# yanrui89/LearningAgileFlight_SE3

Hardware: AMD Instinct MI355X
Metric: MPC solves+gradients/sec (batch, 50-step horizon) at 1/2/4/8 MI355X (higher is better)
Workload: dtype f64

## Files before the change

### learningagileflight_se3_amd/csrc/ipm_kernel.hip

```cpp
#include <hip/hip_runtime.h>

#include <cstdint>

#include "lafse3.h"
#include "model.hpp"
#include "weight_columns.hpp"
#include "riccati_tables.hpp"

namespace lafse3 {

typedef __attribute__((address_space(1))) double gdouble;
typedef double dvec2 __attribute__((ext_vector_type(2)));
typedef __attribute__((address_space(1))) dvec2 gdvec2;

constexpr int MAXN = LAFSE3_MAX_N;
constexpr int SX = MAXN + 1;
constexpr int PST = 18;
constexpr int GST = 22;
constexpr int FMAX = 64;
constexpr int WAVE = 64;
__device__ inline int lane_id() { return (int)(threadIdx.x & (WAVE - 1)); }
__device__ inline int64_t slot_id() { return (int64_t)blockIdx.x; }
constexpr int TRACE_W = 16;
constexpr int DUMP_STEP_W = (MAXN + 1) * NX + MAXN * NU + MAXN * NX;
constexpr int DUMP_W = 2 * DUMP_STEP_W + 2 * MAXN * NU + 2 * (MAXN + 1) * 3;
static_assert(DUMP_W == 3732, "lafse3.h documents the dump record as 3732 doubles per instance");
constexpr int RD_STEP_W = DUMP_STEP_W + 2 * MAXN * NX;
constexpr int RD_POINT_W = DUMP_W - DUMP_STEP_W + 4 * MAXN * NX;
constexpr int RD_REF_W = (MAXN + 1) * NX + MAXN * NU;
constexpr int RD_NSCAL = 6;
constexpr int RD_SCAL = RD_STEP_W + RD_POINT_W + RD_REF_W;
constexpr int RD_LSQ = RD_SCAL + RD_NSCAL;
constexpr int RD_W = RD_LSQ + MAXN * NX + 2;
static_assert(RD_W == 9153, "lafse3.h documents the restoration dump record as 9153 doubles per instance");

enum Mode : int { MODE_SOLVE = 0, MODE_OBJECTIVE = 1, MODE_GRAD = 2, MODE_GETINPUT = 3, MODE_REWARD = 4 };
enum { ST_SOLVED = 0, ST_ACCEPTABLE = 1, ST_MAXITER = 2, ST_LS_FAIL = 3, ST_NONFINITE = 4, ST_TINY = 5,
       ST_REG_FAIL = 6, ST_DEVICE_ERR = 7, ST_RESTO_FAIL = 8, ST_INFEASIBLE = 9 };
constexpr int CNT_ERR = 4;
constexpr int CNT_RESTO = 5;
constexpr int N_COUNTERS = 7;
enum : unsigned long long { ERR_PROBE_LOST = 1ull };

constexpr int WS_RQ = 0;
constexpr int WS_RR = WS_RQ + NX * SX;
constexpr int WS_RC = WS_RR + NU * SX;
constexpr int WS_BDX = WS_RC + NX * SX;
constexpr int WS_BDU = WS_BDX + NX * SX;
constexpr int WS_BLP = WS_BDU + NU * SX;
constexpr int BK_DX = 0, BK_DU = WS_BDU - WS_BDX, BK_LP = WS_BLP - WS_BDX;
constexpr int WS_TAB = WS_BLP + NX * SX;
constexpr int PSTR = NUP17 + 1;
constexpr int WS_PST = WS_TAB + MAXN * TB_W;
constexpr int WS_PN = WS_PST + MAXN * PSTR;
constexpr int WS_Z = WS_PN + 16;
constexpr int WS_CS = WS_Z + 14 * SX;
constexpr int WS_SDX = WS_CS + NX * SX;
constexpr int WS_SDU = WS_SDX + NX * SX;
constexpr int WS_SLP = WS_SDU + NU * SX;
constexpr int RC_K = 0, RC_KF = 4 * NA, RC_L = RC_KF + NU, REC = RC_L + 10;
static_assert(REC % 2 == 0, "record: whole 16-byte pieces");
constexpr int WS_REC = (WS_SLP + NX * SX + 1) & ~1;
constexpr int WS_KREF = WS_REC + MAXN * REC;
constexpr int WS_GS = WS_KREF + NU * SX;
constexpr int WS_PC = WS_GS + NU * SX;
constexpr int WS_RADJ = WS_PC + (MAXN + 1) * 18;
constexpr int WS_PVK = WS_RADJ + (MAXN + 1) * 16;
constexpr int WS_DX = WS_PVK + (MAXN + 1) * 18;
constexpr int WS_DU = WS_DX + NX * SX;
constexpr int WS_LAM = WS_DU + NU * SX;
constexpr int WS_LAMP = WS_LAM + NX * SX;
constexpr int WS_FILT = WS_LAMP + NX * SX;
#ifdef LAFSE3_FAC_CHECK
constexpr int WS_CHK = WS_FILT + 2 * FMAX;
constexpr int WS_END = WS_CHK + MAXN * (REC + PSTR) + (MAXN + 1) * 18;
#else
constexpr int WS_END = WS_FILT + 2 * FMAX;
#endif
constexpr int WS_SIZE0 = (WS_END + 15) & ~15;
constexpr int WS_SIZE = ((WS_SIZE0 / 16) % 2 == 0) ? WS_SIZE0 + 16 : WS_SIZE0;
constexpr int R_P = 0, R_N = R_P + NX * SX, R_ZP = R_N + NX * SX, R_ZN = R_ZP + NX * SX;
constexpr int R_DP = R_ZN + NX * SX, R_DN = R_DP + NX * SX, R_RP = R_DN + NX * SX, R_RN = R_RP + NX * SX;
constexpr int R_BP = R_RN + NX * SX, R_BN = R_BP + NX * SX, R_D = R_BN + NX * SX, R_C = R_D + NX * SX;
constexpr int R_XR = R_C + NX * SX, R_DX2 = R_XR + NX * SX, R_UR = R_DX2 + NX * SX, R_DU2 = R_UR + NU * SX;
constexpr int R_SLAM = R_DU2 + NU * SX, R_SZ = R_SLAM + NX * SX, R_FILT = R_SZ + 14 * SX;
constexpr int RS_L = 0, RS_SD = 91, RS_PK = RS_SD + NX, RS_PV = RS_PK + 91, RS_K = RS_PV + NX, RS_KF = RS_K + NU * NX;
constexpr int RS_STG = RS_KF + NU;
constexpr int R_STG = R_FILT + 2 * FMAX;
constexpr int R_WD = R_STG + MAXN * RS_STG;
constexpr int WD_X = 0, WD_U = WD_X + NX * SX, WD_LAM = WD_U + NU * SX, WD_Z = WD_LAM + NX * SX, WD_DX = WD_Z + 14 * SX;
constexpr int WD_DU = WD_DX + NX * SX, WD_LP = WD_DU + NU * SX, WD_SIZE = WD_LP + NX * SX;
constexpr int RWS_SIZE = (R_WD + WD_SIZE + 15) & ~15;
constexpr int RW_SIZE = 768;
constexpr int WS_ZLU = WS_Z, WS_ZUU = WS_Z + NU * SX, WS_ZLW = WS_Z + 2 * NU * SX, WS_ZUW = WS_Z + 2 * NU * SX + 3 * SX;
#define WS_TRAJ(ws)                                                                                          \
    [[maybe_unused]] double *DX = const_cast<double *>(S.dx), *DU = const_cast<double *>(S.du);              \
    [[maybe_unused]] double *LAM = const_cast<double *>(S.lam), *LP = const_cast<double *>(S.lamp);          \
    [[maybe_unused]] gdouble *ZLU = (gdouble *)(ws) + WS_ZLU, *ZUU = (gdouble *)(ws) + WS_ZUU;                 \
    [[maybe_unused]] gdouble *ZLW = (gdouble *)(ws) + WS_ZLW, *ZUW = (gdouble *)(ws) + WS_ZUW

struct KernelArgs {
    lafse3_params prm;
    int mode;
    int64_t n_inst;
    const double *ini, *goal, *gate12, *ptra, *atra, *t, *ulast;
    const float *dnn;
    const double *x_in;
    double *x_out, *u_out, *lam_out, *cost_out, *reward_out;
    int32_t *status_out, *iters_out;
    unsigned long long *counters;
    int persistent;
    unsigned *sched;
    double *trace;
    int trace_iters;
    unsigned long long *ptime;
    double *dump;
    int dump_it;
    int dump_refine;
    int64_t drop_push;
    double *ws;
    double *rws;
};

struct RestoDumpArgs {
    double *buf;
    int entry, it;
    int refine;
};
constexpr int REC_X = 0, REC_U = REC_X + (MAXN + 1) * NX, REC_LAM = REC_U + MAXN * NU, REC_ZLU = REC_LAM + MAXN * NX;
constexpr int REC_ZUU = REC_ZLU + MAXN * NU, REC_ZLW = REC_ZUU + MAXN * NU, REC_ZUW = REC_ZLW + (MAXN + 1) * 3;
constexpr int REC_MU = REC_ZUW + (MAXN + 1) * 3, REC_S = REC_MU + 1, REC_STATUS = REC_S + 1, REC_N = REC_STATUS + 1;
constexpr int REC_W = REC_N + 1;
static_assert(REC_MU == DUMP_W - DUMP_STEP_W, "the record's arrays are dump_point's iterate block");
static_assert(REC_W == 2223, "lafse3.h documents the optimum record as 2223 doubles per instance");
struct ExtArgs {
    const double *weights;
    double *dx_out, *du_out;
    double *gain_out;
    int32_t *sens_out;
    int32_t groups;
    double *rec;
};

struct Ctl {
    int N;
    double s;
    double mu;
    double ulo, uhi, wlo, whi;
};

constexpr int RING = 24;
constexpr int VGU = 44;
struct __align__(16) Smem {
    double x[NX * SX], u[NU * SX];
    double dx[NX * SX], du[NU * SX];
    double lam[NX * SX], lamp[NX * SX];
    alignas(16) double P[NA * PST];
    double p[24];
    union {
// ... 569 lines not shown
        double nr = 0.0;
        for (int r = 0; r < 1; ++r) nr = kkt_residual(M, at, S, C, ws, dw, soc);
        PT_END(S, 6);
        if (step < 0) {
            ratio = nr;
            ratios[0] = nr; ratios[1] = -1; ratios[2] = -1; ratios[3] = 0;
            continue;
        }
        if (step < 2) ratios[1 + step] = nr;
        ratios[3] += 1;
        if (!(nr < ratio)) {
            revert_to_backup(DX, LP, DU, bk, C.N);
            vm_sync();
            break;
        }
        ratio = nr;
    }
    return 1;
}

__device__ __noinline__ void soc_defects(const Model &M, const Smem &S, const Ctl &C, gdouble *ws, double alpha, int init)
{
    WS_TRAJ(ws);
    const int lane = lane_id();
    const int N = C.N;
    gdouble *cs = ws + WS_CS;
    if (lane < N) {
        const int k = lane;
        double xk[NX], uk[NU], xn[NX];
#pragma unroll
        for (int i = 0; i < NX; ++i) xk[i] = S.x[i * SX + k] + alpha * DX[i * SX + k];
#pragma unroll
        for (int a = 0; a < NU; ++a) uk[a] = S.u[a * SX + k] + alpha * DU[a * SX + k];
        f_disc(M, xk, uk, xn);
#pragma unroll
        for (int i = 0; i < NX; ++i) {
            const double ct = xn[i] - (S.x[i * SX + k + 1] + alpha * DX[i * SX + k + 1]);
            cs[i * SX + k] = init ? ct : alpha * cs[i * SX + k] + ct;
        }
    }
    vm_sync();
}

__device__ __noinline__ void soc_direction(const Model &M, const Attitude &at, Smem &S, const Ctl &C, gdouble *ws,
                                           double dw, int &sweeps)
{
    const int lane = lane_id();
    const int N = C.N;
    gdouble *rq = ws + WS_RQ, *rr = ws + WS_RR, *rc = ws + WS_RC;
    const gdouble *cs = ws + WS_CS;
    if (lane < N) {
        const int k = lane;
        double gu[NU];
        grad_u(M, S, C, k, gu);
#pragma unroll
        for (int a = 0; a < NU; ++a) {
            double gb, sg;
            bar_terms(S.u[a * SX + k], C.ulo, C.uhi, 0, 0, C.mu, gb, sg);
            rr[a * SX + k] = gu[a] + gb;
        }
        const int k1 = k + 1;
        double x1[NX], g[NX];
        load_stage(S, k1, x1);
        grad_x(M, at, S, C, k1, x1, g);
#pragma unroll
        for (int c = 0; c < 3; ++c) {
            double gb, sg;
            bar_terms(x1[10 + c], C.wlo, C.whi, 0, 0, C.mu, gb, sg);
            g[10 + c] += gb;
        }
#pragma unroll
        for (int i = 0; i < NX; ++i) {
            rq[i * SX + k1] = g[i];
            rc[i * SX + k] = cs[i * SX + k];
        }
    }
    vm_sync();
    double ratios[4] = {0, 0, 0, 0};
    linear_solve(M, at, S, C, ws, dw, 0, 0, 1, 1, sweeps, ratios, nullptr);
}

struct BoundDir {
    double du[NU], zlu[NU], zuu[NU], dw[3], zlw[3], zuw[3];
};
__device__ __attribute__((always_inline)) inline void load_bound_dir(const Smem &S, gdouble *ws, int k, BoundDir &b)
{
    WS_TRAJ(ws);
    const int k1 = k + 1;
#pragma unroll
    for (int a = 0; a < NU; ++a) {
        b.du[a] = DU[a * SX + k];
        b.zlu[a] = ZLU[a * SX + k];
        b.zuu[a] = ZUU[a * SX + k];
    }
#pragma unroll
    for (int c = 0; c < 3; ++c) {
        b.dw[c] = DX[(10 + c) * SX + k1];
        b.zlw[c] = ZLW[c * SX + k1];
        b.zuw[c] = ZUW[c * SX + k1];
    }
    __builtin_amdgcn_sched_barrier(0);
}

__device__ __noinline__ void frac_to_bound(const Smem &S, const Ctl &C, gdouble *ws, double tau, double mu, double &amax,
                                           double &az)
{
    WS_TRAJ(ws);
    const int lane = lane_id();
    const int N = C.N;
    double am = 1.0, a_z = 1.0;
    if (lane < N) {
        const int k = lane;
        const int k1 = k + 1;
        BoundDir bd;
        load_bound_dir(S, ws, k, bd);
#pragma unroll
        for (int a = 0; a < NU; ++a) {
            double v = S.u[a * SX + k], d = bd.du[a];
            double sl = v - C.ulo, su = C.uhi - v;
            if (d < 0) am = fmin(am, -tau * sl / d);
            if (d > 0) am = fmin(am, tau * su / d);
            double zl = bd.zlu[a], zu = bd.zuu[a];
            double dzl = mu / sl - zl - zl / sl * d;
            double dzu = mu / su - zu + zu / su * d;
            if (dzl < 0) a_z = fmin(a_z, -tau * zl / dzl);
            if (dzu < 0) a_z = fmin(a_z, -tau * zu / dzu);
        }
#pragma unroll
        for (int c = 0; c < 3; ++c) {
            double v = S.x[(10 + c) * SX + k1], d = bd.dw[c];
            double sl = v - C.wlo, su = C.whi - v;
            if (d < 0) am = fmin(am, -tau * sl / d);
            if (d > 0) am = fmin(am, tau * su / d);
            double zl = bd.zlw[c], zu = bd.zuw[c];
            double dzl = mu / sl - zl - zl / sl * d;
            double dzu = mu / su - zu + zu / su * d;
            if (dzl < 0) a_z = fmin(a_z, -tau * zl / dzl);
            if (dzu < 0) a_z = fmin(a_z, -tau * zu / dzu);
        }
    }
    amax = wmin(am);
    az = wmin(a_z);
}

struct DirStats {
    double amax, az, gBD, rel;
};
__device__ __noinline__ DirStats direction_stats(const Model &M, const Attitude &at, const Smem &S, const Ctl &C, gdouble *ws,
                                                 double tau, double mu)
{
    WS_TRAJ(ws);
    const int lane = lane_id();
    const int N = C.N;
double amax = 1.0, az = 1.0, gBD = 0.0, rel = 0.0;
    if (lane < N) {
        const int k = lane;
        BoundDir bd;
        load_bound_dir(S, ws, k, bd);
        double gu[NU];
        grad_u(M, S, C, k, gu);
#pragma unroll
        for (int a = 0; a < NU; ++a) {
            double v = S.u[a * SX + k], d = bd.du[a];
            double sl = v - C.ulo, su = C.uhi - v;
            if (d < 0) amax = fmin(amax, -tau * sl / d);
            if (d > 0) amax = fmin(amax, tau * su / d);
            double zl = bd.zlu[a], zu = bd.zuu[a];
            double dzl = mu / sl - zl - zl / sl * d;
            double dzu = mu / su - zu + zu / su * d;
            if (dzl < 0) az = fmin(az, -tau * zl / dzl);
            if (dzu < 0) az = fmin(az, -tau * zu / dzu);
            double gb, sg;
            bar_terms(v, C.ulo, C.uhi, 0, 0, mu, gb, sg);
            gBD += (gu[a] + gb) * d;
            rel = fmax(rel, fabs(d) / (1.0 + fabs(v)));
        }
        const int k1 = k + 1;
        double x1[NX], g[NX];
        load_stage(S, k1, x1);
        grad_x(M, at, S, C, k1, x1, g);
#pragma unroll
        for (int c = 0; c < 3; ++c) {
            double v = x1[10 + c], d = bd.dw[c];
            double sl = v - C.wlo, su = C.whi - v;
            if (d < 0) amax = fmin(amax, -tau * sl / d);
            if (d > 0) amax = fmin(amax, tau * su / d);
            double zl = bd.zlw[c], zu = bd.zuw[c];
            double dzl = mu / sl - zl - zl / sl * d;
            double dzu = mu / su - zu + zu / su * d;
            if (dzl < 0) az = fmin(az, -tau * zl / dzl);
            if (dzu < 0) az = fmin(az, -tau * zu / dzu);
            double gb, sg;
            bar_terms(v, C.wlo, C.whi, 0, 0, mu, gb, sg);
            g[10 + c] += gb;
        }
#pragma unroll
        for (int i = 0; i < NX; ++i) {
            double d = DX[i * SX + k1];
            gBD += g[i] * d;
            rel = fmax(rel, fabs(d) / (1.0 + fabs(x1[i])));
        }
    }
    amax = wmin(amax);
    az = wmin(az);
    gBD = wsum(gBD);
    rel = wmax(rel);
    DirStats D;
    D.amax = amax;
    D.az = az;
    D.gBD = gBD;
    D.rel = rel;
    return D;
}

__device__ __noinline__ void accept_step(Smem &S, const Ctl &C, gdouble *ws, double alpha, double az, double mu)
{
    WS_TRAJ(ws);
    const int lane = lane_id();
    const int N = C.N;
    if (lane < N) {
        const int k = lane, k1 = k + 1;
        double zlu_[NU], zuu_[NU], zlw_[3], zuw_[3];
#pragma unroll
        for (int a = 0; a < NU; ++a) {
            zlu_[a] = ZLU[a * SX + k];
            zuu_[a] = ZUU[a * SX + k];
        }
#pragma unroll
        for (int c = 0; c < 3; ++c) {
            zlw_[c] = ZLW[c * SX + k1];
            zuw_[c] = ZUW[c * SX + k1];
        }
#pragma unroll
        for (int a = 0; a < NU; ++a) {
            double v = S.u[a * SX + k], d = DU[a * SX + k];
            double sl = v - C.ulo, su = C.uhi - v;
            double zl = zlu_[a], zu = zuu_[a];
            zl = zl + az * (mu / sl - zl - zl / sl * d);
            zu = zu + az * (mu / su - zu + zu / su * d);
            v = v + alpha * d;
            S.u[a * SX + k] = v;
            sl = v - C.ulo;
            su = C.uhi - v;
            zlu_[a] = fmax(fmin(zl, 1e10 * mu / sl), mu / (1e10 * sl));
            zuu_[a] = fmax(fmin(zu, 1e10 * mu / su), mu / (1e10 * su));
        }
#pragma unroll
        for (int c = 0; c < 3; ++c) {
            double v = S.x[(10 + c) * SX + k1], d = DX[(10 + c) * SX + k1];
            double sl = v - C.wlo, su = C.whi - v;
            double zl = zlw_[c], zu = zuw_[c];
            zlw_[c] = zl + az * (mu / sl - zl - zl / sl * d);
            zuw_[c] = zu + az * (mu / su - zu + zu / su * d);
        }
        double lk[NX], lpk[NX], dx1[NX];
#pragma unroll
        for (int i = 0; i < NX; ++i) {
            lk[i] = LAM[i * SX + k];
            lpk[i] = LP[i * SX + k];
            dx1[i] = DX[i * SX + k1];
        }
#pragma unroll
        for (int i = 0; i < NX; ++i) {
            LAM[i * SX + k] = lk[i] + alpha * (lpk[i] - lk[i]);
            S.x[i * SX + k1] += alpha * dx1[i];
        }
#pragma unroll
        for (int c = 0; c < 3; ++c) {
            double v = S.x[(10 + c) * SX + k1];
            double sl = v - C.wlo, su = C.whi - v;
            double zl = zlw_[c], zu = zuw_[c];
            zlw_[c] = fmax(fmin(zl, 1e10 * mu / sl), mu / (1e10 * sl));
            zuw_[c] = fmax(fmin(zu, 1e10 * mu / su), mu / (1e10 * su));
        }
#pragma unroll
        for (int a = 0; a < NU; ++a) {
            ZLU[a * SX + k] = zlu_[a];
            ZUU[a * SX + k] = zuu_[a];
        }
#pragma unroll
        for (int c = 0; c < 3; ++c) {
            ZLW[c * SX + k1] = zlw_[c];
            ZUW[c * SX + k1] = zuw_[c];
        }
    }
    vm_sync();
}

static_assert(FMAX <= WAVE, "one filter entry per lane");
__device__ inline int filter_ok(const gdouble *FT, const gdouble *FP, int nfilt, double th, double ph)
{
    const int f = opaque_lane();
    double ft = 0.0, fp = 0.0;
    if (f < nfilt) {
        ft = FT[f];
        fp = FP[f];
    }
    return __ballot(f < nfilt && !(th <= ft || ph <= fp)) == 0ull;
}
__device__ inline int filter_add(gdouble *FT, gdouble *FP, int nfilt, double th0, double ph0)
{
    const int lane = opaque_lane();
    const double nt = (1.0 - 1e-5) * th0, np = ph0 - 1e-8 * th0;
    double ft = 0.0, fp = 0.0;
    if (lane < nfilt) {
        ft = FT[lane];
        fp = FP[lane];
    }
    const bool keep = lane < nfilt && !(ft >= nt && fp >= np);
    const unsigned long long m = __ballot(keep);
    int w = __popcll(m);
    if (keep) {
        const int pos = __popcll(m & ((1ull << lane) - 1ull));
        FT[pos] = ft;
        FP[pos] = fp;
    }
    if (w < FMAX) {
        if (lane == 0) {
            FT[w] = nt;
            FP[w] = np;
        }
        w++;
    }
    vm_sync();
    return w;
}

__device__ inline int ls_accept(const gdouble *FT, const gdouble *FP, int nfilt, double alpha_test, double tht, double pht, int okt, double th0,
                                double ph0, double gBD, double pg, double pt, double theta_max, double theta_min)
{
    const double eps = 2.220446049250313e-16;
    int acc = okt && !(tht > theta_max);
    if (acc) {
        int ftype = (gBD < 0) && (alpha_test * pg > pt);
        if (ftype && th0 <= theta_min) {
            acc = (pht - ph0 - 1e-8 * alpha_test * gBD) <= 10.0 * eps * fabs(ph0);
        } else {
            int objinc_ok = 1;
            if (pht > ph0) {
                double basval = (fabs(ph0) > 10.0) ? log10(fabs(ph0)) : 1.0;
                if (log10(pht - ph0) > 5.0 + basval) objinc_ok = 0;
            }
            acc = objinc_ok && (((tht - (1.0 - 1e-5) * th0) <= 10.0 * eps * fabs(th0)) ||
                                ((pht - ph0 + 1e-8 * th0) <= 10.0 * eps * fabs(ph0)));
        }
    }
    if (acc && !filter_ok(FT, FP, nfilt, tht, pht)) return 0;
    return acc;
}
__device__ inline int ls_accept(const gdouble *FT, const gdouble *FP, int nfilt, double alpha_test, double tht, double pht, int okt, double th0,
                                double ph0, double gBD, double theta_max, double theta_min)
{
    double pg = 0.0, pt = 0.0;
    if (okt && !(tht > theta_max) && gBD < 0) {
        pg = pow(-gBD, 2.3);
        pt = pow(th0, 1.1);
    }
    return ls_accept(FT, FP, nfilt, alpha_test, tht, pht, okt, th0, ph0, gBD, pg, pt, theta_max, theta_min);
}

struct Errs {
    double dinf, pinf, cmu, c0, sd, sc;
};

__device__ __attribute__((always_inline)) inline Errs compute_errors(const Model &M, const Attitude &at, const Smem &S, const Ctl &C, gdouble *ws,
                                            double mu)
{
    Errs E;
    WS_TRAJ(ws);
    const int lane = opaque_lane();
    const int N = C.N;
    double dinf = 0, pinf = 0, cmu = 0, c0 = 0, smult = 0, sz = 0;
    if (lane < N) {
        const int k = lane;
        double xk[NX], uk[NU], lk[NX];
        load_stage(S, k, xk);
        load_u(S, k, uk);
#pragma unroll
        for (int i = 0; i < NX; ++i) lk[i] = LAM[i * SX + k];
        double gu[NU], btl[NU];
        grad_u(M, S, C, k, gu);
        Bt_times(M, xk, lk, btl);
#pragma unroll
        for (int a = 0; a < NU; ++a) {
            double zl = ZLU[a * SX + k], zu = ZUU[a * SX + k];
            double acc = gu[a] + btl[a] - zl + zu;
            dinf = fmax(dinf, fabs(acc));
            double sl = uk[a] - C.ulo, su = C.uhi - uk[a];
            cmu = fmax(cmu, fmax(fabs(sl * zl - mu), fabs(su * zu - mu)));
            c0 = fmax(c0, fmax(fabs(sl * zl), fabs(su * zu)));
            sz += zl + zu;
        }
        double xn[NX];
        f_disc(M, xk, uk, xn);
#pragma unroll
        for (int i = 0; i < NX; ++i) {
            pinf = fmax(pinf, fabs(xn[i] - S.x[i * SX + k + 1]));
            smult += fabs(lk[i]);
        }
        const int k1 = k + 1;
        double x1[NX], g[NX];
        load_stage(S, k1, x1);
        grad_x(M, at, S, C, k1, x1, g);
#pragma unroll
        for (int i = 0; i < NX; ++i) g[i] -= lk[i];
        if (k1 < N) {
            double u1[NU], l1[NX], atl[NX];
            load_u(S, k1, u1);
#pragma unroll
            for (int i = 0; i < NX; ++i) l1[i] = LAM[i * SX + k1];
            At_times(M, x1, u1, l1, atl);
#pragma unroll
            for (int i = 0; i < NX; ++i) g[i] += atl[i];
        }
#pragma unroll
        for (int c = 0; c < 3; ++c) {
            double zl = ZLW[c * SX + k1], zu = ZUW[c * SX + k1];
            g[10 + c] += -zl + zu;
            double sl = x1[10 + c] - C.wlo, su = C.whi - x1[10 + c];
            cmu = fmax(cmu, fmax(fabs(sl * zl - mu), fabs(su * zu - mu)));
            c0 = fmax(c0, fmax(fabs(sl * zl), fabs(su * zu)));
            sz += zl + zu;
        }
#pragma unroll
        for (int i = 0; i < NX; ++i) dinf = fmax(dinf, fabs(g[i]));
    }
    dinf = wmax(dinf);
    pinf = wmax(pinf);
    cmu = wmax(cmu);
    c0 = wmax(c0);
    smult = wsum(smult);
    sz = wsum(sz);
    const double smax = 100.0;
    double n_mult = (double)(N * NX) + (double)(N * NU * 2 + N * 3 * 2);
    double n_z = (double)(N * NU * 2 + N * 3 * 2);
    E.sd = fmax(smax, (smult + sz) / n_mult) / smax;
    E.sc = fmax(smax, sz / n_z) / smax;
    E.dinf = dinf;
    E.pinf = pinf;
    E.cmu = cmu;
    E.c0 = c0;
    return E;
}

__device__ inline double err_value(const Errs &E, int with_mu)
{
    double c = with_mu ? E.cmu : E.c0;
    return fmax(E.dinf / E.sd, fmax(E.pinf, c / E.sc));
}

struct Merit {
    double theta, phi;
    int ok;
    double J, lb;
};
__device__ __attribute__((always_inline)) inline Merit eval_merit(const Model &M, const Attitude &at, const Smem &S, const Ctl &C, gdouble *ws,
                                         double alpha, double mu)
{
    WS_TRAJ(ws);
    const int lane = opaque_lane();
    const int N = C.N;
    double th = 0, lb = 0, J = 0;
    int good = 1;
    if (lane < N) {
        const int k = lane;
        double xk[NX], x1[NX], uk[NU], up[NU];
#pragma unroll
        for (int i = 0; i < NX; ++i) {
            xk[i] = S.x[i * SX + k] + alpha * DX[i * SX + k];
            x1[i] = S.x[i * SX + k + 1] + alpha * DX[i * SX + k + 1];
        }
#pragma unroll
        for (int a = 0; a < NU; ++a) {
            uk[a] = S.u[a * SX + k] + alpha * DU[a * SX + k];
            up[a] = (k == 0) ? S.ulast[a] : S.u[a * SX + k - 1] + alpha * DU[a * SX + k - 1];
        }
        double xn[NX];
        f_disc(M, xk, uk, xn);
#pragma unroll
        for (int i = 0; i < NX; ++i) th += fabs(xn[i] - x1[i]);
        double pu = 1.0, pw = 1.0, su_[NU], sl_[NU], sw_[3], sv_[3];
#pragma unroll
        for (int a = 0; a < NU; ++a) {
            sl_[a] = uk[a] - C.ulo; su_[a] = C.uhi - uk[a];
            if (!(sl_[a] > 0) || !(su_[a] > 0)) good = 0;
            pu *= sl_[a] * su_[a];
        }
#pragma unroll
        for (int c = 0; c < 3; ++c) {
            const double v = x1[10 + c];
            sv_[c] = v - C.wlo; sw_[c] = C.whi - v;
            if (!(sv_[c] > 0) || !(sw_[c] > 0)) good = 0;
            pw *= sv_[c] * sw_[c];
        }
        if (pu > 1e-290 && pu < 1e290 && pw > 1e-290 && pw < 1e290) {
            lb = log(pu) + log(pw);
        } else {
#pragma unroll
            for (int a = 0; a < NU; ++a) lb += log(sl_[a]) + log(su_[a]);
#pragma unroll
            for (int c = 0; c < 3; ++c) lb += log(sv_[c]) + log(sw_[c]);
        }
        double c = state_cost(M, at, S.goal, S.ptra, S.wk[k], xk);
        double thr = 0, sm = 0;
#pragma unroll
        for (int a = 0; a < NU; ++a) {
            thr += uk[a] * uk[a];
            sm += (uk[a] - up[a]) * (uk[a] - up[a]);
        }
        c += M.wthrust * thr + M.du_w * sm;
        if (k == N - 1) c += state_cost(M, at, S.goal, S.ptra, 0.0, x1);
        J = c;
    }
    th = wsum(th);
    lb = wsum(lb);
    J = wsum(J);
    good = wand(good);
    Merit R;
    R.theta = th;
    R.phi = C.s * J - mu * lb;
    R.ok = good && isfinite(R.phi) && isfinite(th);
    R.J = J;
    R.lb = lb;
    return R;
}

__device__ __noinline__ double pd_error(const Model &M, const Attitude &at, const Smem &S, const Ctl &C, gdouble *ws,
                                        double alpha, double mu)
{
    WS_TRAJ(ws);
    const int lane = lane_id();
    const int N = C.N;
    double dual = 0, primal = 0, cmpl = 0;
    if (lane < N) {
        const int k = lane, k1 = k + 1;
        auto ut = [&](int a, int kk) { return S.u[a * SX + kk] + alpha * DU[a * SX + kk]; };
        auto lt = [&](int i, int kk) { return LAM[i * SX + kk] + alpha * (LP[i * SX + kk] - LAM[i * SX + kk]); };
        double xk[NX], uk[NU], lk[NX], x1[NX];
#pragma unroll
        for (int i = 0; i < NX; ++i) {
            xk[i] = S.x[i * SX + k] + alpha * DX[i * SX + k];
            x1[i] = S.x[i * SX + k1] + alpha * DX[i * SX + k1];
            lk[i] = lt(i, k);
        }
#pragma unroll
        for (int a = 0; a < NU; ++a) uk[a] = ut(a, k);
        double btl[NU];
        Bt_times(M, xk, lk, btl);
#pragma unroll
        for (int a = 0; a < NU; ++a) {
            const double up = (k == 0) ? S.ulast[a] : ut(a, k - 1);
            double g = 2 * M.wthrust * uk[a] + M.du_w * 2 * (uk[a] - up);
            if (k + 1 < N) g += -M.du_w * 2 * (ut(a, k + 1) - uk[a]);
            g *= C.s;
            const double v = S.u[a * SX + k], d = DU[a * SX + k];
            const double sl = v - C.ulo, su = C.uhi - v;
            const double zl0 = ZLU[a * SX + k], zu0 = ZUU[a * SX + k];
            const double zl = zl0 + alpha * (mu / sl - zl0 - zl0 / sl * d);
            const double zu = zu0 + alpha * (mu / su - zu0 + zu0 / su * d);
            dual += fabs(g + btl[a] - zl + zu);
            cmpl += fabs((uk[a] - C.ulo) * zl - mu) + fabs((C.uhi - uk[a]) * zu - mu);
        }
        double xn[NX];
        f_disc(M, xk, uk, xn);
#pragma unroll
        for (int i = 0; i < NX; ++i) primal += fabs(xn[i] - x1[i]);
        double g[NX];
        grad_x(M, at, S, C, k1, x1, g);
#pragma unroll
        for (int i = 0; i < NX; ++i) g[i] -= lk[i];
        if (k1 < N) {
            double u1[NU], l1[NX], atl[NX];
#pragma unroll
            for (int a = 0; a < NU; ++a) u1[a] = ut(a, k1);
#pragma unroll
            for (int i = 0; i < NX; ++i) l1[i] = lt(i, k1);
            At_times(M, x1, u1, l1, atl);
#pragma unroll
            for (int i = 0; i < NX; ++i) g[i] += atl[i];
        }
#pragma unroll
        for (int c = 0; c < 3; ++c) {
            const double v = S.x[(10 + c) * SX + k1], d = DX[(10 + c) * SX + k1];
            const double sl = v - C.wlo, su = C.whi - v;
            const double zl0 = ZLW[c * SX + k1], zu0 = ZUW[c * SX + k1];
            const double zl = zl0 + alpha * (mu / sl - zl0 - zl0 / sl * d);
            const double zu = zu0 + alpha * (mu / su - zu0 + zu0 / su * d);
            g[10 + c] += -zl + zu;
            cmpl += fabs((x1[10 + c] - C.wlo) * zl - mu) + fabs((C.whi - x1[10 + c]) * zu - mu);
        }
#pragma unroll
        for (int i = 0; i < NX; ++i) dual += fabs(g[i]);
    }
    return wsum(dual + primal + cmpl);
}
// ... 455 lines not shown
        double pl = fmin(1e-2 * fmax(1.0, fabs(C.ulo)), 1e-2 * (C.uhi - C.ulo));
        double pu = fmin(1e-2 * fmax(1.0, fabs(C.uhi)), 1e-2 * (C.uhi - C.ulo));
        double uinit = fmin(fmax(umid, C.ulo + pl), C.uhi - pu);
        pl = fmin(1e-2 * fmax(1.0, fabs(C.wlo)), 1e-2 * (C.whi - C.wlo));
        pu = fmin(1e-2 * fmax(1.0, fabs(C.whi)), 1e-2 * (C.whi - C.wlo));
        double winit = fmin(fmax(wmid, C.wlo + pl), C.whi - pu);
        if (lane <= N) {
            const int k = lane;
#pragma unroll
            for (int i = 0; i < NX; ++i) {
                double v = 0.0;
                if (k == 0) v = A.ini[b * NX + i];
                else if (i >= 10) v = winit;
                S.x[i * SX + k] = v;
                DX[i * SX + k] = 0.0;
            }
#pragma unroll
            for (int c = 0; c < 3; ++c) {
                ZLW[c * SX + k] = (k >= 1) ? 1.0 : 0.0;
                ZUW[c * SX + k] = (k >= 1) ? 1.0 : 0.0;
            }
            double dtk = prm.dt * k - tt;
            if constexpr (EXT) S.wk[k] = w_peak * exp(-w_decay * dtk * dtk);
            else S.wk[k] = prm.tra_w_peak * exp(-prm.tra_w_decay * dtk * dtk);
        }
        if (lane < N) {
            const int k = lane;
#pragma unroll
            for (int a = 0; a < NU; ++a) {
                S.u[a * SX + k] = uinit;
                ZLU[a * SX + k] = 1.0;
                ZUU[a * SX + k] = 1.0;
                DU[a * SX + k] = 0.0;
            }
#pragma unroll
            for (int i = 0; i < NX; ++i) {
                LAM[i * SX + k] = 0.0;
                LP[i * SX + k] = 0.0;
            }
        }
    }
    if constexpr (WARM)
        if (warm)
            warm_load_primal(S, wrec, A.ini + b * NX, ZW->shift, ZW->bound_push, ZW->bound_frac, prm.dt, tt, w_peak,
                             w_decay);
    init_gv_const(M, S);
    vm_sync();
    {
        double gm = 0.0;
        if (lane < N) {
            double g[NX], x1[NX], gu[NU];
            load_stage(S, lane + 1, x1);
            grad_x(M, at, S, C, lane + 1, x1, g);
#pragma unroll
            for (int i = 0; i < NX; ++i) gm = fmax(gm, fabs(g[i]));
            grad_u(M, S, C, lane, gu);
#pragma unroll
            for (int a = 0; a < NU; ++a) gm = fmax(gm, fabs(gu[a]));
        }
        gm = wmax(gm);
        if (gm > 100.0) C.s = fmax(100.0 / gm, 1e-8);
    }
    int iters = 0, sweeps = 0, trials = 0;
    if constexpr (WARM)
        if (warm) {
            warm_load_duals(S, ws, wrec, ZW->shift, C.s / wrec[REC_S], ZW->mult_bound_push);
            vm_sync();
        }
    if (prm.lsq_mult_init && !warm) {
        double rat[4];
        int ok = linear_solve(M, at, S, C, ws, 0.0, 1, 1, 0, 0, sweeps, rat, nullptr);
        if (ok) {
            double mx = 0.0;
            if (lane < N)
#pragma unroll
                for (int i = 0; i < NX; ++i) mx = fmax(mx, fabs(LP[i * SX + lane]));
            mx = wmax(mx);
            if (mx <= 1e3 && lane < N)
#pragma unroll
                for (int i = 0; i < NX; ++i) LAM[i * SX + lane] = LP[i * SX + lane];
        }
        vm_sync();
    }

    double mu = C.mu;
    double tau = fmax(0.99, 1.0 - mu);
    int nfilt = 0;
    double theta_max = -1, theta_min = -1;
    double dw_last = 0.0;
    int acc_count = 0;
    int status = ST_MAXITER;
    int tiny_flag = 0;
    int in_soft_resto = 0, soft_resto_counter = 0;
    int resto_entries = 0, resto_returns = 0;
    int in_wd = 0, wd_short = 0, wd_trial = 0;
    double wd_th = 0.0, wd_ph = 0.0, wd_gBD = 0.0;
    bool have_m0 = false;
    double m0_theta = 0.0, m0_J = 0.0, m0_lb = 0.0;
    const double eps = 2.220446049250313e-16;

    PT_END(S, 0);
#ifdef LAFSE3_FACBENCH
#ifndef LAFSE3_FACBENCH_REFINE
#define LAFSE3_FACBENCH_REFINE 1
#endif
    for (int r = 0; r < LAFSE3_FACBENCH; ++r) {
        double rat[4];
        linear_solve(M, at, S, C, ws, 1e-2, 1, 0, LAFSE3_FACBENCH_REFINE, 0, sweeps, rat, nullptr);
    }
    iters = LAFSE3_FACBENCH;
    constexpr int ipm_on = 0;
#else
    constexpr int ipm_on = 1;
#endif
    int it = 0;
    for (;;) {
    int resto_req = 0;
    double r_th0 = 0.0, r_ph0 = 0.0, r_e0 = 0.0;
    for (; ipm_on && it <= prm.max_iter; ++it) {
        Errs E = compute_errors(M, at, S, C, ws, mu);
        PT_END(S, 1);
        double e0 = err_value(E, 0);
        if (!isfinite(e0)) { status = ST_NONFINITE; break; }
        if constexpr (EXT)
            if (w_nonfinite) { status = ST_NONFINITE; break; }
        if (e0 <= prm.tol && E.dinf / C.s <= 1.0 && E.pinf <= 1e-4 && E.c0 / C.s <= 1e-4) {
            status = ST_SOLVED;
            break;
        }
        if (e0 <= prm.acceptable_tol && E.dinf / C.s <= 1e10 && E.pinf <= 1e-2 && E.c0 / C.s <= 1e-2) {
            if (++acc_count >= prm.acceptable_iter) { status = ST_ACCEPTABLE; break; }
        } else {
            acc_count = 0;
        }
        if (it == prm.max_iter) { status = ST_MAXITER; break; }
        {
            const double mu_min = prm.tol / 10.0;
            int done_tiny = 0;
            for (;;) {
                double emu = err_value(E, 1);
                if (!(emu <= 10.0 * mu || tiny_flag)) break;
                double nmu = fmax(mu_min, fmin(0.2 * mu, pow15(mu)));
                if (nmu == mu) {
                    if (tiny_flag) done_tiny = 1;
                    break;
                }
                mu = nmu;
                tau = fmax(0.99, 1.0 - mu);
                nfilt = 0;
                in_soft_resto = 0;
                in_wd = 0;
                wd_short = 0;
                tiny_flag = 0;
                E = compute_errors(M, at, S, C, ws, mu);
            }
            PT_END(S, 1);
            if (done_tiny) { status = ST_TINY; break; }
            C.mu = mu;
        }
        PT_END(S, 11);
        double dw = 0.0;
        double ratios[4] = {0, 0, 0, 0};
        if constexpr (DUMP)
            if (A.dump && it == A.dump_it) dump_point(S, ws, N, A.dump + inst * (int64_t)DUMP_W + DUMP_STEP_W);
        double *dpre = (A.dump && it == A.dump_it && !A.dump_refine) ? A.dump + inst * (int64_t)DUMP_W : nullptr;
        int ok = linear_solve(M, at, S, C, ws, 0.0, 1, 0, 1, 0, sweeps, ratios, dpre);
        if (!ok) {
            dw = (dw_last == 0.0) ? 1e-4 : fmax(1e-20, dw_last / 3.0);
            for (;;) {
                ok = linear_solve(M, at, S, C, ws, dw, 2, 0, 1, 0, sweeps, ratios, dpre);
                if (ok) { dw_last = dw; break; }
                dw *= (dw_last == 0.0) ? 100.0 : 8.0;
                if (dw > 1e40) break;
            }
            if (!ok) { status = ST_REG_FAIL; break; }
        }
        if (A.dump && it == A.dump_it && A.dump_refine) dump_step(S, ws, N, A.dump + inst * (int64_t)DUMP_W);
        PT_RESTART();
        const DirStats D = direction_stats(M, at, S, C, ws, tau, mu);
        PT_LS(0);
        double amax = D.amax, gBD = D.gBD;
        const double rel = D.rel;
        double az = D.az;
        double th0, ph0, j0, lb0;
        if (have_m0) {
            th0 = m0_theta;
            ph0 = C.s * m0_J - mu * m0_lb;
            j0 = m0_J;
            lb0 = m0_lb;
        } else {
            const Merit m0 = eval_merit(M, at, S, C, ws, 0.0, mu);
            th0 = m0.theta;
            ph0 = m0.phi;
            j0 = m0.J;
            lb0 = m0.lb;
        }
        have_m0 = false;
        PT_LS(1);
        double tJ = 0.0, tlb = 0.0;
        if (theta_max < 0) {
            theta_max = uniform(1e4 * fmax(1.0, th0));
            theta_min = uniform(1e-4 * fmax(1.0, th0));
        }
        int accepted = 0, soc_taken = 0;
        int is_tiny = (rel < 10.0 * eps) && (th0 <= 1e-4);
        double rth = th0, rph = ph0, rgBD = gBD;
        int skip_first = 0;
        gdouble *rs = (gdouble *)(A.rws + slot_id() * (int64_t)RWS_SIZE);
        if (__builtin_expect(in_wd && is_tiny, 0)) {
            wd_copy(S, ws, rs, 0);
            in_wd = 0;
            wd_short = 0;
            rth = th0 = wd_th;
            rph = ph0 = wd_ph;
            rgBD = gBD = wd_gBD;
            frac_to_bound(S, C, ws, tau, mu, amax, az);
            is_tiny = 0;
            skip_first = 2;
        }
        if (__builtin_expect(prm.watchdog > 0 && !in_wd && !is_tiny && !in_soft_resto && wd_short >= prm.watchdog, 0)) {
            wd_copy(S, ws, rs, 1);
            wd_th = th0;
            wd_ph = ph0;
            wd_gBD = gBD;
            wd_trial = 0;
            in_wd = 1;
        }
        const int wd_ref = in_wd && !is_tiny && !in_soft_resto;
        double pw_g = 0.0, pw_t = 0.0;
        if (gBD < 0 && !is_tiny && !wd_ref) {
            pw_g = pow(-gBD, 2.3);
            pw_t = pow(th0, 1.1);
        }
        double alpha = amax, alpha_test = amax;
        double tht = 0, pht = 0;
        int soft_step = 0;
        int wd_step = 0, n_rej = 0;
        auto try_soft = [&]() {
            const double as = fmin(amax, az);
            const double cur = pd_error(M, at, S, C, ws, 0.0, mu);
            const double trial = pd_error(M, at, S, C, ws, as, mu);
            const Merit mt = eval_merit(M, at, S, C, ws, as, mu);
            trials++;
            if (!(trial <= 0.9999 * cur)) return;
            accepted = 1;
            tht = mt.theta;
            pht = mt.phi;
            tJ = mt.J;
            tlb = mt.lb;
            soft_step = 1 + ls_accept(FT, FP, nfilt, 0.0, tht, pht, mt.ok, th0, ph0, gBD, pw_g, pw_t, theta_max, theta_min);
            alpha = az = alpha_test = as;
        };
        if (is_tiny) {
            accepted = 1;
            tiny_flag = 1;
        } else if (in_soft_resto) {
            if (++soft_resto_counter <= 10) {
                try_soft();
                if (soft_step == 2) { in_soft_resto = 0; soft_resto_counter = 0; }
            }
        } else {
            if (in_wd) {
                rth = wd_th;
                rph = wd_ph;
                rgBD = wd_gBD;
                if (rgBD < 0) {
                    pw_g = pow(-rgBD, 2.3);
                    pw_t = pow(rth, 1.1);
                }
                const Merit mt = eval_merit(M, at, S, C, ws, amax, mu);
                trials++;
                tht = mt.theta;
                pht = mt.phi;
                tJ = mt.J;
                tlb = mt.lb;
                if (ls_accept(FT, FP, nfilt, amax, tht, pht, mt.ok, rth, rph, rgBD, pw_g, pw_t, theta_max, theta_min)) {
                    accepted = 1;
                    in_wd = 0;
                } else if (++wd_trial > 3) {
                    wd_copy(S, ws, rs, 0);
                    in_wd = 0;
                    wd_short = 0;
                    rth = th0 = wd_th;
                    rph = ph0 = wd_ph;
                    rgBD = gBD = wd_gBD;
                    frac_to_bound(S, C, ws, tau, mu, amax, az);
                    skip_first = 1;
                } else {
                    accepted = 1;
                    wd_step = 1;
                }
                alpha = alpha_test = amax;
            }
            double amin_base = 1e-5;
            if (gBD < 0) {
                amin_base = fmin(1e-5, 1e-8 * th0 / (-gBD));
                if (th0 <= theta_min) amin_base = fmin(amin_base, pw_t / pw_g);
            }
            const double alpha_min = 0.05 * amin_base;
            if (skip_first == 1) alpha = 0.5 * amax;
            for (int n_steps = 0; !accepted; ++n_steps) {
                n_rej = n_steps;
                int okt;
                PT_LS(5);
                {
                    const Merit mt = eval_merit(M, at, S, C, ws, alpha, mu);
                    tht = mt.theta;
// ... 425 lines not shown
```

Before: 9593.

## Skip exact tiny-step measure and full error recompute when provably unnecessary

In direction_stats, each lane now checks with a cheap test whether any component clearly exceeds the tiny-step threshold, and a wave ballot chooses that path. Only when no lane proves the step is large does the code compute the exact relative step measure, which needs reloads and divisions. In the mu-update loop, only the complementarity error is recomputed for the new mu instead of calling the full compute_errors, because dual and primal infeasibility do not depend on mu. This relies on rel only being compared against the tiny threshold and on the other error terms being unchanged, so any later use of the exact rel value or of the skipped sd/sc terms could change behaviour.

```diff
diff --git a/learningagileflight_se3_amd/csrc/exact_skips.hpp b/learningagileflight_se3_amd/csrc/exact_skips.hpp
--- /dev/null
+++ b/learningagileflight_se3_amd/csrc/exact_skips.hpp
@@ -0,0 +1,35 @@
+#pragma once
+#ifndef __host__
+#define __host__
+#define __device__
+#endif
+#include <cmath>
+
+#ifndef LAFSE3_EXACT_SKIPS
+#define LAFSE3_EXACT_SKIPS 1
+#endif
+#ifndef LAFSE3_XS_B
+#define LAFSE3_XS_B LAFSE3_EXACT_SKIPS
+#endif
+#ifndef LAFSE3_XS_D
+#define LAFSE3_XS_D LAFSE3_EXACT_SKIPS
+#endif
+
+namespace lafse3 {
+namespace xs {
+
+constexpr bool ON_B = LAFSE3_XS_B != 0, ON_D = LAFSE3_XS_D != 0;
+constexpr double INF = __builtin_huge_val();
+constexpr double TINY_C = 10.0 * 2.220446049250313e-16;
+constexpr double REL_NOT_TINY = 1.0;
+
+__host__ __device__ inline bool proves_not_tiny(double d, double v)
+{
+    if (!ON_B) return false;
+    const double w = 1.0 + fabs(v);
+    return fabs(d) >= (2.0 * TINY_C) * w && w < INF;
+}
+__host__ __device__ inline double tiny_measure(double rel, double d, double v) { return fmax(rel, fabs(d) / (1.0 + fabs(v))); }
+
+}
+}
diff --git a/learningagileflight_se3_amd/csrc/ipm_kernel.hip b/learningagileflight_se3_amd/csrc/ipm_kernel.hip
--- a/learningagileflight_se3_amd/csrc/ipm_kernel.hip
+++ b/learningagileflight_se3_amd/csrc/ipm_kernel.hip
@@ -5,6 +5,7 @@
 #include "lafse3.h"
 #include "model.hpp"
 #include "weight_columns.hpp"
+#include "exact_skips.hpp"
 #include "riccati_tables.hpp"
 
 namespace lafse3 {
@@ -880,7 +881,8 @@
     WS_TRAJ(ws);
     const int lane = lane_id();
     const int N = C.N;
-double amax = 1.0, az = 1.0, gBD = 0.0, rel = 0.0;
+    double amax = 1.0, az = 1.0, gBD = 0.0, rel = 0.0;
+    bool big = false;
     if (lane < N) {
         const int k = lane;
         BoundDir bd;
@@ -901,7 +903,7 @@
             double gb, sg;
             bar_terms(v, C.ulo, C.uhi, 0, 0, mu, gb, sg);
             gBD += (gu[a] + gb) * d;
-            rel = fmax(rel, fabs(d) / (1.0 + fabs(v)));
+            big |= xs::proves_not_tiny(d, v);
         }
         const int k1 = k + 1;
         double x1[NX], g[NX];
@@ -926,13 +928,24 @@
         for (int i = 0; i < NX; ++i) {
             double d = DX[i * SX + k1];
             gBD += g[i] * d;
-            rel = fmax(rel, fabs(d) / (1.0 + fabs(x1[i])));
+            big |= xs::proves_not_tiny(d, x1[i]);
         }
     }
     amax = wmin(amax);
     az = wmin(az);
     gBD = wsum(gBD);
-    rel = wmax(rel);
+    if (__ballot(big) != 0ull) {
+        rel = xs::REL_NOT_TINY;
+    } else {
+        if (lane < N) {
+            const int k = lane, k1 = k + 1;
+#pragma unroll
+            for (int a = 0; a < NU; ++a) rel = xs::tiny_measure(rel, DU[a * SX + k], S.u[a * SX + k]);
+#pragma unroll
+            for (int i = 0; i < NX; ++i) rel = xs::tiny_measure(rel, DX[i * SX + k1], S.x[i * SX + k1]);
+        }
+        rel = wmax(rel);
+    }
     DirStats D;
     D.amax = amax;
     D.az = az;
@@ -1169,6 +1182,31 @@
     E.cmu = cmu;
     E.c0 = c0;
     return E;
+}
+
+__device__ __attribute__((always_inline)) inline double compl_error_mu(const Smem &S, const Ctl &C, gdouble *ws, double mu)
+{
+#pragma clang fp contract(off)
+    WS_TRAJ(ws);
+    const int lane = opaque_lane();
+    const int N = C.N;
+    double cmu = 0;
+    if (lane < N) {
+        const int k = lane, k1 = k + 1;
+#pragma unroll
+        for (int a = 0; a < NU; ++a) {
+            const double zl = ZLU[a * SX + k], zu = ZUU[a * SX + k], v = S.u[a * SX + k];
+            const double sl = v - C.ulo, su = C.uhi - v;
+            cmu = fmax(cmu, fmax(fabs(fma(sl, zl, -mu)), fabs(fma(su, zu, -mu))));
+        }
+#pragma unroll
+        for (int c = 0; c < 3; ++c) {
+            const double zl = ZLW[c * SX + k1], zu = ZUW[c * SX + k1], v = S.x[(10 + c) * SX + k1];
+            const double sl = v - C.wlo, su = C.whi - v;
+            cmu = fmax(cmu, fmax(fabs(fma(sl, zl, -mu)), fabs(fma(su, zu, -mu))));
+        }
+    }
+    return wmax(cmu);
 }
 
 __device__ inline double err_value(const Errs &E, int with_mu)
@@ -1930,7 +1968,10 @@
                 in_wd = 0;
                 wd_short = 0;
                 tiny_flag = 0;
-                E = compute_errors(M, at, S, C, ws, mu);
+                if constexpr (xs::ON_D)
+                    E.cmu = compl_error_mu(S, C, ws, mu);
+                else
+                    E = compute_errors(M, at, S, C, ws, mu);
             }
             PT_END(S, 1);
             if (done_tiny) { status = ST_TINY; break; }
```

After: 9589. No clear change (-0.0%).
